# jaronlong52/neuron_poker

Hardware: NVIDIA B200
Metric: showdown_evals_per_s (higher is better)
Workload: dtype u32

## Files before the change

neuron_poker_b200/csrc/npk_device.cuh:

```cuda
#pragma once
#include <cuda_runtime.h>
#include <stdint.h>

namespace npk {

constexpr int kDevDescShift = 9;
constexpr int kRowBits = 10;
constexpr uint32_t kColMask = (1u << kRowBits) - 1u;

struct DeviceTables {
    const uint16_t* value;
    const uint16_t* rowoff;
    const uint16_t* flush;
    const uint32_t* desc;
    uint32_t value_bytes;
    uint32_t rowoff_bytes;
    uint32_t flush_bytes;
    uint16_t type_start[10];
    uint32_t* check;
};

struct SmemTables {
    const uint16_t* value;
    const uint16_t* rowoff;
    const uint16_t* flush;
    const uint32_t* desc;
    uint32_t value_bytes, rowoff_bytes, flush_bytes;
    uint32_t* check;
};

#ifdef NPK_CHECKED
#define NPK_CHECK(ptr, cond, code) do { if (!(cond)) atomicMax((ptr), (unsigned)(code)); } while (0)
#else
#define NPK_CHECK(ptr, cond, code) do { } while (0)
#endif

constexpr uint32_t kDescBytes = 256;

__device__ __forceinline__ uint32_t smem_u32(const void* p) { return (uint32_t)__cvta_generic_to_shared(p); }

__device__ __forceinline__ void mbar_init(uint64_t* bar, uint32_t count)
{
    asm volatile("mbarrier.init.shared::cta.b64 [%0], %1;" ::"r"(smem_u32(bar)), "r"(count));
    asm volatile("fence.mbarrier_init.release.cluster;" ::: "memory");
}
__device__ __forceinline__ void mbar_expect_tx(uint64_t* bar, uint32_t bytes)
{
    asm volatile("mbarrier.arrive.expect_tx.shared::cta.b64 _, [%0], %1;" ::"r"(smem_u32(bar)), "r"(bytes) : "memory");
}
__device__ __forceinline__ void bulk_g2s(void* dst, const void* src, uint32_t bytes, uint64_t* bar)
{
    asm volatile("cp.async.bulk.shared::cluster.global.mbarrier::complete_tx::bytes [%0], [%1], %2, [%3];" ::"r"(
                     smem_u32(dst)),
                 "l"(src), "r"(bytes), "r"(smem_u32(bar))
                 : "memory");
}
__device__ __forceinline__ void mbar_wait(uint64_t* bar, uint32_t parity)
{
    uint32_t done = 0;
    while (!done) {
        asm volatile(
            "{\n .reg .pred p;\n mbarrier.try_wait.parity.shared::cta.b64 p, [%1], %2;\n selp.u32 %0, 1, 0, p;\n}\n"
            : "=r"(done)
            : "r"(smem_u32(bar)), "r"(parity)
            : "memory");
    }
}

__device__ __forceinline__ SmemTables stage_tables(const DeviceTables& t, uint8_t* base, uint64_t* bar)
{
    uint8_t* s_value = base;
    uint8_t* s_rowoff = s_value + t.value_bytes;
    uint8_t* s_flush = s_rowoff + t.rowoff_bytes;
    if (threadIdx.x == 0) mbar_init(bar, 1);
    __syncthreads();
    if (threadIdx.x == 0) {
        mbar_expect_tx(bar, t.value_bytes + t.rowoff_bytes + t.flush_bytes + kDescBytes);
        const uint32_t kChunk = 32768;
        for (uint32_t o = 0; o < t.value_bytes; o += kChunk)
            bulk_g2s(s_value + o, (const uint8_t*)t.value + o, min(kChunk, t.value_bytes - o), bar);
        bulk_g2s(s_rowoff, t.rowoff, t.rowoff_bytes, bar);
        bulk_g2s(s_flush, t.flush, t.flush_bytes, bar);
        bulk_g2s(s_flush + t.flush_bytes, t.desc, kDescBytes, bar);
    }
    mbar_wait(bar, 0);
    SmemTables s;
    s.value = (const uint16_t*)s_value;
    s.rowoff = (const uint16_t*)s_rowoff;
    s.flush = (const uint16_t*)s_flush;
    s.desc = (const uint32_t*)(s_flush + t.flush_bytes);
    s.value_bytes = t.value_bytes; s.rowoff_bytes = t.rowoff_bytes; s.flush_bytes = t.flush_bytes; s.check = t.check;
    return s;
}

__device__ __forceinline__ void philox4x32_10(uint32_t c0, uint32_t c1, uint32_t c2, uint32_t c3, uint32_t k0,
                                              uint32_t k1, uint32_t out[4])
{
    const uint32_t M0 = 0xD2511F53u, M1 = 0xCD9E8D57u, W0 = 0x9E3779B9u, W1 = 0xBB67AE85u;
#pragma unroll
    for (int r = 0; r < 10; r++) {
        uint64_t p0 = (uint64_t)M0 * c0, p1 = (uint64_t)M1 * c2;
        uint32_t n0 = (uint32_t)(p1 >> 32) ^ c1 ^ k0;
        uint32_t n2 = (uint32_t)(p0 >> 32) ^ c3 ^ k1;
        c1 = (uint32_t)p1;
        c3 = (uint32_t)p0;
        c0 = n0;
        c2 = n2;
        k0 += W0;
        k1 += W1;
    }
    out[0] = c0; out[1] = c1; out[2] = c2; out[3] = c3;
}

__device__ __forceinline__ uint32_t prmt(uint32_t a, uint32_t b, uint32_t sel)
{
    uint32_t r;
    asm("prmt.b32 %0, %1, %2, %3;" : "=r"(r) : "r"(a), "r"(b), "r"(sel));
    return r;
}

__device__ __forceinline__ uint32_t shr_clamp(uint32_t v, uint32_t n)
{
    uint32_t r;
    asm("shr.u32 %0, %1, %2;" : "=r"(r) : "r"(v), "r"(n));
    return r;
}

__device__ __forceinline__ uint32_t lds_u16(uint32_t saddr)
{
    uint32_t v;
    asm("ld.shared.u16 %0, [%1];" : "=r"(v) : "r"(saddr));
    return v;
}

struct SmemAddr {
    uint32_t value, rowoff, flush;
#ifdef NPK_CHECKED
    uint32_t value_bytes, rowoff_bytes, flush_bytes;
    uint32_t* check;
#endif
};

__device__ __forceinline__ SmemAddr smem_addr(const SmemTables& s)
{
    SmemAddr a;
    a.value = smem_u32(s.value); a.rowoff = smem_u32(s.rowoff); a.flush = smem_u32(s.flush);
#ifdef NPK_CHECKED
    a.value_bytes = s.value_bytes; a.rowoff_bytes = s.rowoff_bytes; a.flush_bytes = s.flush_bytes; a.check = s.check;
#endif
    return a;
}

__device__ __forceinline__ uint32_t lookup_nonflush(const SmemAddr& a, uint32_t total)
{
    const uint32_t row2 = __umulhi(total, 1u << (32 - (kDevDescShift + kRowBits - 1))) & (0xFFFFu << 1);
    NPK_CHECK(a.check, row2 + 2u <= a.rowoff_bytes, 1);
    const uint32_t off = lds_u16(a.rowoff + row2);
    const uint32_t col2 = __umulhi(total, 1u << (32 - (kDevDescShift - 1))) & (kColMask << 1);
    NPK_CHECK(a.check, col2 + (off << 1) + 2u <= a.value_bytes, 2);
    return lds_u16(a.value + col2 + (off << 1));
}

__device__ __forceinline__ uint32_t flush_bit(uint32_t d, uint32_t fsx) { return shr_clamp(0x1000u, (d ^ fsx) & 63u); }

__device__ __forceinline__ void card_bits(uint32_t d, uint32_t& lo, uint32_t& hi)
{
    const uint64_t b = 1ull << ((d & 0x30u) + 12u - (d & 15u));
    lo = (uint32_t)b;
    hi = (uint32_t)(b >> 32);
}

__device__ __forceinline__ uint32_t suit_inc(uint32_t d) { return 1u << ((d >> 2) & 12u); }

__device__ __forceinline__ uint32_t field_selector(uint32_t fs) { return 0x9910u + fs * 0x2222u; }

__device__ __forceinline__ uint32_t eval7_desc(const SmemAddr& a, const uint32_t d[7])
{
    uint32_t total = 0, cnt = 0x3333u;
#pragma unroll
    for (int i = 0; i < 7; i++) {
        total += d[i];
        cnt += suit_inc(d[i]);
    }
    uint32_t v = lookup_nonflush(a, total);
    const uint32_t f = cnt & 0x8888u;
    if (f) {
        const uint32_t fsx = (((31u - __clz(f)) >> 2) & 3u) << 4;
        uint32_t field = 0;
#pragma unroll
        for (int i = 0; i < 7; i++) field |= shr_clamp(0x1000u, (d[i] ^ fsx) & 63u);
        NPK_CHECK(a.check, 2u * field + 2u <= a.flush_bytes, 3);
        v = lds_u16(a.flush + 2u * field);
    }
    return v;
}

}
```

neuron_poker_b200/csrc/npk_mc.cuh:

```cuda
#pragma once
#include "npk_device.cuh"
#include "npk_kernels.h"

namespace npk {

__device__ __forceinline__ long long next_item(unsigned long long* counter, int lane)
{
    unsigned long long it = 0;
    if (lane == 0) it = atomicAdd(counter, 1ull);
    return (long long)__shfl_sync(0xffffffffu, it, 0);
}

__device__ __forceinline__ void item_range(const EquityParams& p, long long item, long long& qslot, long long& begin, long long& end)
{
    qslot = item / p.chunks;
    begin = (item - qslot * p.chunks) * p.chunk;
    end = min(p.trials, begin + (long long)p.chunk);
}

struct QueryStatic {
    uint32_t hero_sum;
    uint32_t hero_lo, hero_hi;
    uint32_t board_sum;
    uint32_t board_lo, board_hi;
    uint32_t board_cnt;
    uint64_t known;
};

__device__ __forceinline__ QueryStatic load_query(const EquityParams& p, const uint32_t* sdesc, long long q, int nb_known)
{
    QueryStatic s;
    const uint8_t h0 = p.hole ? p.hole[2 * q] : (uint8_t)p.inline_query;
    const uint8_t h1 = p.hole ? p.hole[2 * q + 1] : (uint8_t)(p.inline_query >> 8);
    uint32_t d0 = sdesc[h0], d1 = sdesc[h1], l, h;
    s.hero_sum = d0 + d1;
    card_bits(d0, s.hero_lo, s.hero_hi);
    card_bits(d1, l, h);
    s.hero_lo |= l; s.hero_hi |= h;
    s.known = (1ull << h0) | (1ull << h1);
    s.board_sum = 0; s.board_lo = 0; s.board_hi = 0; s.board_cnt = 0x5555u;
    for (int i = 0; i < nb_known; i++) {
        const uint8_t c = p.hole ? p.board[5 * q + i] : (uint8_t)(p.inline_query >> (16 + 8 * i));
        uint32_t d = sdesc[c];
        card_bits(d, l, h);
        s.board_sum += d; s.board_lo |= l; s.board_hi |= h; s.board_cnt += suit_inc(d);
        s.known |= 1ull << c;
    }
    return s;
}

__device__ __forceinline__ void finish_single_call(const EquityParams& p, int lane)
{
    SingleCall* sc = p.single;
    if (!sc) return;
    __syncwarp();
    unsigned int last = 0;
    if (lane == 0) {
        __threadfence();
        const unsigned int total = gridDim.x * (blockDim.x >> 5);
        last = atomicAdd(&sc->ticket, 1u) == total - 1u;
    }
    last = __shfl_sync(0xffffffffu, last, 0);
    if (!last) return;
    __threadfence();
    unsigned long long v = 0;
    if (lane < 12) {
        unsigned long long* src = &sc->wins;
        v = atomicExch(src + lane, 0ull);
    }
    if (lane == 0) { sc->work_counter = 0; sc->ticket = 0; }
    if (p.single_quick) {
        const unsigned long long t = __shfl_sync(0xffffffffu, v, 1);
        if (lane == 0) {
            const uint4 q = make_uint4((unsigned int)v, (unsigned int)t, (unsigned int)p.single_seq, (unsigned int)(p.single_seq >> 32));
            asm volatile("st.global.v4.u32 [%0], {%1, %2, %3, %4};" ::"l"(&sc->host->quick), "r"(q.x), "r"(q.y), "r"(q.z), "r"(q.w)
                         : "memory");
        }
        return;
    }
    if (lane < 12) (&sc->host->wins)[lane] = v;
    __threadfence_system();
    __syncwarp();
    if (lane == 0) *reinterpret_cast<volatile unsigned long long*>(&sc->host->seq) = p.single_seq;
}

static __device__ __noinline__ void finish_peer(PeerCall* pc, unsigned long long epoch, unsigned long long* totals, uint32_t words,
                                         int lane)
{
    __syncwarp();
    unsigned int last = 0;
    if (lane == 0) {
        __threadfence();
        const unsigned int total = gridDim.x * (blockDim.x >> 5);
        last = atomicAdd(&pc->ticket, 1u) == total - 1u;
    }
    last = __shfl_sync(0xffffffffu, last, 0);
    if (!last) return;
    __threadfence();
    const uint32_t world = pc->world, me = pc->rank;
    const uint32_t parity = (uint32_t)(epoch & 1ull);
    const size_t my_slot = ((size_t)parity * world + me) * pc->stride;
    for (uint32_t base = 0; base < words; base += 128) {
        unsigned long long v[4];
#pragma unroll
        for (int k = 0; k < 4; k++) {
            const uint32_t i = base + 32u * k + lane;
            v[k] = i < words ? atomicExch(&pc->acc[i], 0ull) : 0ull;
        }
        for (uint32_t r = 0; r < world; r++) {
            unsigned long long* dst = pc->slots[r] + my_slot;
#pragma unroll
            for (int k = 0; k < 4; k++) {
                const uint32_t i = base + 32u * k + lane;
                if (i < words) dst[i] = v[k];
            }
        }
    }
    __threadfence_system();
    __syncwarp();
    if (lane < world)
        asm volatile("st.release.sys.global.u64 [%0], %1;" ::"l"(pc->flags[lane] + parity * kMaxPeers + me), "l"(epoch) : "memory");
    if (lane < world) {
        const unsigned long long* f = pc->flags[me] + parity * kMaxPeers + lane;
        const long long t0 = clock64();
        unsigned long long seen;
        for (;;) {
            asm volatile("ld.acquire.sys.global.u64 %0, [%1];" : "=l"(seen) : "l"(f) : "memory");
            if (seen >= epoch) break;
            if (clock64() - t0 > (4ll << 30)) { pc->error = 1u; break; }
        }
    }
    __syncwarp();
    const unsigned long long* mine = pc->slots[me] + (size_t)parity * world * pc->stride;
    for (uint32_t base = 0; base < words; base += 128) {
        unsigned long long sum[4] = {0, 0, 0, 0};
#pragma unroll 4
        for (uint32_t r = 0; r < world; r++) {
#pragma unroll
            for (int k = 0; k < 4; k++) {
                const uint32_t i = base + 32u * k + lane;
                if (i < words) sum[k] += __ldcg(mine + (size_t)r * pc->stride + i);
            }
        }
#pragma unroll
        for (int k = 0; k < 4; k++) {
            const uint32_t i = base + 32u * k + lane;
            if (i < words) totals[i] = sum[k];
        }
    }
    if (lane == 0) { pc->work_counter = 0; pc->ticket = 0; }
}

struct BoardFlush {
    uint32_t fsx;
    uint32_t sel;
    uint32_t thr;
};

__device__ __forceinline__ BoardFlush board_flush(uint32_t board_cnt)
{
    BoardFlush b;
    const uint32_t f = board_cnt & 0x8888u;
    const uint32_t fs = ((31u - __clz(f)) >> 2) & 3u;
    b.fsx = fs << 4;
    b.sel = field_selector(fs);
    b.thr = f ? 5u : 64u;
    return b;
}

__device__ __forceinline__ uint32_t eval_player(const SmemAddr& a, uint32_t total, uint32_t field, uint32_t thr)
{
    uint32_t v = lookup_nonflush(a, total);
    NPK_CHECK(a.check, 2u * field + 2u <= a.flush_bytes, 3);
    if ((uint32_t)__popc(field) >= thr) v = max(v, lds_u16(a.flush + 2u * field));
    return v;
}

__device__ __forceinline__ uint32_t lds_u32(uint32_t saddr)
{
    uint32_t v;
    asm volatile("ld.shared.u32 %0, [%1];" : "=r"(v) : "r"(saddr) : "memory");
    return v;
}
__device__ __forceinline__ void sts_u32(uint32_t saddr, uint32_t v)
{
    asm volatile("st.shared.u32 [%0], %1;" ::"r"(saddr), "r"(v) : "memory");
}

struct WarpCtx {
    SmemAddr st;
    const uint32_t* sdesc;
    uint32_t* scratch;
    uint32_t fy_addr;
    int lane;
};

__device__ __forceinline__ WarpCtx warp_context(const EquityParams& p, uint8_t* smem, int words_per_warp)
{
    uint64_t* bar = reinterpret_cast<uint64_t*>(smem);
    const SmemTables stab = stage_tables(p.tables, smem + 128, bar);
    const uint32_t table_bytes = 128 + p.tables.value_bytes + p.tables.rowoff_bytes + p.tables.flush_bytes + kDescBytes;
    const int warp = threadIdx.x >> 5, lane = threadIdx.x & 31;
    WarpCtx cx;
    cx.st = smem_addr(stab);
    cx.sdesc = stab.desc;
    cx.scratch = reinterpret_cast<uint32_t*>(smem + table_bytes) + warp * words_per_warp;
    cx.fy_addr = smem_u32(cx.scratch + 64 + lane);
    cx.lane = lane;
    return cx;
}

template <int NOPP, int NB>
__device__ __forceinline__ void uniform_item(const EquityParams& p, const WarpCtx& cx, long long q, long long t_begin,
            long long t_end)
{
    constexpr int KNOWN = 5 - NB;
    constexpr int N = 50 - KNOWN;
    constexpr int D = 2 * NOPP + NB;
    constexpr int NW = (D + 1) / 2;
    constexpr int NBLK2 = (2 * NW + 3) / 4;
    static_assert(D <= N, "not enough cards");

    const SmemAddr& st = cx.st;
    const int lane = cx.lane;
    uint32_t* scratch = cx.scratch;
    uint32_t* fy = scratch + 64 + lane;
    const uint32_t fy_addr = cx.fy_addr;
    const QueryStatic qs = load_query(p, cx.sdesc, q, KNOWN);

    __syncwarp();
    {
        const uint64_t avail = ~qs.known & ((1ull << 52) - 1ull);
        for (int c = lane; c < 52; c += 32)
            if (avail >> c & 1ull) scratch[__popcll(avail & ((1ull << c) - 1ull))] = cx.sdesc[c];
    }
    __syncwarp();
#pragma unroll 4
    for (int j = 0; j < N; j++) fy[j * 32] = scratch[j];
    __syncwarp();

    const unsigned long long a_begin = (unsigned long long)(p.trial_offset + t_begin);
    const unsigned long long a_end = (unsigned long long)(p.trial_offset + t_end);
    uint32_t wins = 0, ties = 0;
    unsigned long long wt_pack = 0;

    const uint32_t span = (uint32_t)(a_end - a_begin);
    uint32_t rel = (uint32_t)(2ull * (a_begin >> 1) - a_begin) + 2u * (uint32_t)lane;
    for (unsigned long long pb = a_begin >> 1; pb <= (a_end - 1) >> 1; pb += 32, rel += 64u) {
        const unsigned long long pair = pb + lane;
        uint32_t w[NBLK2 > 0 ? NBLK2 * 4 : 1];
#pragma unroll
        for (int b = 0; b < NBLK2; b++)
            philox4x32_10((uint32_t)pair, (uint32_t)(pair >> 32), (uint32_t)q + p.query_offset, (uint32_t)b,
                          p.seed_lo, p.seed_hi, &w[4 * b]);
        uint32_t dv[2][D > 0 ? D : 1];
#pragma unroll
        for (int u = 0; u < 2; u++) {
            uint32_t slot[D > 0 ? D : 1];
            uint32_t rem = 0;
#pragma unroll
            for (int k = 0; k < D; k++) {
                const uint32_t x = (k & 1) ? rem : w[u * NW + (k >> 1)];
                const uint32_t idx = __umulhi(x, (uint32_t)(N - k));
                rem = x * (uint32_t)(N - k);
                slot[k] = fy_addr + idx * 128u;
                dv[u][k] = lds_u32(slot[k]);
                sts_u32(slot[k], lds_u32(fy_addr + (uint32_t)(N - 1 - k) * 128u));
            }
#pragma unroll
            for (int k = D - 1; k >= 0; k--) sts_u32(slot[k], dv[u][k]);
        }
#pragma unroll
        for (int u = 0; u < 2; u++) {
            const bool active = rel + (uint32_t)u < span;
            uint32_t bsum = qs.board_sum, bcnt = qs.board_cnt;
#pragma unroll
            for (int k = 2 * NOPP; k < D; k++) { bsum += dv[u][k]; bcnt += suit_inc(dv[u][k]); }
            const BoardFlush bf = board_flush(bcnt);
            uint32_t bfield = prmt(qs.board_lo, qs.board_hi, bf.sel);
#pragma unroll
            for (int k = 2 * NOPP; k < D; k++) bfield |= flush_bit(dv[u][k], bf.fsx);
            const uint32_t hv = eval_player(st, bsum + qs.hero_sum, bfield | prmt(qs.hero_lo, qs.hero_hi, bf.sel), bf.thr);
            uint32_t best = 0;
#pragma unroll
            for (int o = 0; o < NOPP; o++) {
                const uint32_t d0 = dv[u][2 * o], d1 = dv[u][2 * o + 1];
                best = max(best, eval_player(st, bsum + d0 + d1, bfield | flush_bit(d0, bf.fsx) | flush_bit(d1, bf.fsx), bf.thr));
            }
            const bool win = active && (NOPP == 0 || hv > best), tie = active && NOPP > 0 && hv == best;
            wins += win; ties += tie;
            if (p.win_types && (win || tie)) {
                uint32_t ty = 0;
#pragma unroll
                for (int i = 1; i < 9; i++) ty += hv >= p.tables.type_start[i];
                wt_pack += 1ull << (7 * ty);
            }
        }
    }
#ifdef NPK_CHECKED
    __syncwarp();
    for (int j = 0; j < N; j++) NPK_CHECK(st.check, fy[j * 32] == scratch[j], 7);
#endif
    wins = __reduce_add_sync(0xffffffffu, wins);
    ties = __reduce_add_sync(0xffffffffu, ties);
    if (lane == 0) {
        atomicAdd(&p.wins[q], (unsigned long long)wins);
        atomicAdd(&p.ties[q], (unsigned long long)ties);
    }
    if (p.win_types) {
#pragma unroll
        for (int i = 0; i < 9; i++) {
            uint32_t c = __reduce_add_sync(0xffffffffu, (uint32_t)(wt_pack >> (7 * i)) & 127u);
            if (lane == 0 && c) atomicAdd(&p.win_types[9 * q + i], (unsigned long long)c);
        }
    }
}


struct WordStream {
    uint32_t c0, c1, c2, k0, k1, blk, have;
    uint32_t w[4];
    __device__ __forceinline__ uint32_t next()
    {
        if (have == 0) { philox4x32_10(c0, c1, c2, blk++, k0, k1, w); have = 4; }
        const uint32_t r = w[0];
        w[0] = w[1]; w[1] = w[2]; w[2] = w[3];
        have--;
        return r;
    }
};

__device__ __forceinline__ int select_bit(uint64_t m, int k)
{
    uint32_t lo = (uint32_t)m, hi = (uint32_t)(m >> 32);
    int c = __popc(lo), base = 0;
    uint32_t w = lo;
    if (k >= c) { k -= c; w = hi; base = 32; }
#pragma unroll
    for (int s = 16; s >= 1; s >>= 1) {
        const uint32_t lowmask = (1u << s) - 1u;
        const int cl = __popc(w & lowmask);
        if (k >= cl) { k -= cl; w >>= s; base += s; } else { w &= lowmask; }
    }
    return base;
}

#ifndef NPK_IMAD_LEVEL
#define NPK_IMAD_LEVEL 0
#endif
static __constant__ uint32_t c_mul[12] = {1u, 256u, 65536u, 1u << 24, 1u << 25, 128u, 1u << 31, 1u << 23, 1u << 15, 0u, 0u, 0u};

__device__ __forceinline__ uint32_t imad_lo(uint32_t a, uint32_t b, uint32_t c)
{
    uint32_t r;
    asm("mad.lo.u32 %0, %1, %2, %3;" : "=r"(r) : "r"(a), "r"(b), "r"(c));
    return r;
}
__device__ __forceinline__ uint32_t imad_hi(uint32_t a, uint32_t b, uint32_t c)
{
    uint32_t r;
    asm("mad.hi.u32 %0, %1, %2, %3;" : "=r"(r) : "r"(a), "r"(b), "r"(c));
    return r;
}

__device__ __forceinline__ uint32_t bump4(uint32_t x4, uint32_t c, uint32_t h)
{
#if NPK_IMAD_LEVEL >= 2
    const uint32_t t = imad_lo(x4, c_mul[0], c) & h;
#else
    const uint32_t t = (x4 + c) & h;
#endif
#if NPK_IMAD_LEVEL >= 1
    return imad_hi(t, c_mul[4], x4);
#else
    return x4 + (t >> 7);
#endif
}

template <int D>
__device__ __forceinline__ void lehmer_decode(const uint32_t (&raw)[D > 0 ? D : 1], uint32_t (&x4)[(D + 3) / 4 > 0 ? (D + 3) / 4 : 1])
{
    constexpr int G = (D + 3) / 4;
#pragma unroll
    for (int g = 0; g < G; g++) {
        uint32_t v = raw[4 * g];
#pragma unroll
        for (int b = 1; b < 4; b++)
            if (4 * g + b < D) {
#if NPK_IMAD_LEVEL >= 1
                v = imad_lo(raw[4 * g + b], c_mul[b], v);
#else
                v += raw[4 * g + b] << (8 * b);
#endif
            }
        x4[g] = v;
    }
#pragma unroll
    for (int k = D - 2; k >= 0; k--) {
        const uint32_t c = 0x80808080u - raw[k] * 0x01010101u;
#pragma unroll
        for (int g = (k + 1) / 4; g < G; g++) {
            uint32_t h = 0;
#pragma unroll
            for (int b = 0; b < 4; b++)
                if (4 * g + b > k && 4 * g + b < D) h |= 0x80u << (8 * b);
            x4[g] = bump4(x4[g], c, h);
        }
    }
}

__device__ __forceinline__ uint32_t slot_addr(uint32_t x4, int b, uint32_t base)
{
    const uint32_t f = x4 & (0xFFu << (8 * b));
#if NPK_IMAD_LEVEL >= 1
    return b == 0 ? imad_lo(f, c_mul[5], base) : imad_hi(f, c_mul[5 + b], base);
#else
    return b == 0 ? base + f * 128u : base + (f >> (8 * b - 7));
#endif
}

template <int NOPP, int NB>
__device__ __forceinline__ void refdeal_item(const EquityParams& p, const WarpCtx& cx, long long q, long long t_begin,
            long long t_end)
{
    constexpr int KNOWN = 5 - NB;
    constexpr int N = 50 - KNOWN;
    constexpr int D = 2 * NOPP + NB;
#ifdef NPK_UNIFORM_LEHMER
    constexpr int NWR = (D + 1) / 2;
#else
    constexpr int NWR = NOPP + (NB + 1) / 2;
#endif
    constexpr int NBLK2 = (2 * NWR + 3) / 4;
    constexpr int G = (D + 3) / 4;
    static_assert(D <= N, "not enough cards");

    const SmemAddr& st = cx.st;
    const int lane = cx.lane;
    uint32_t* scratch = cx.scratch;
    uint32_t* fy = scratch + 64 + lane;
    const uint32_t fy_addr = cx.fy_addr;
    const QueryStatic qs = load_query(p, cx.sdesc, q, KNOWN);

    __syncwarp();
    {
        const uint64_t avail = ~qs.known & ((1ull << 52) - 1ull);
        for (int c = lane; c < 52; c += 32)
            if (avail >> c & 1ull) scratch[__popcll(avail & ((1ull << c) - 1ull))] = cx.sdesc[c];
    }
    __syncwarp();
#pragma unroll 4
    for (int j = 0; j < N; j++) fy[j * 32] = scratch[j];
    __syncwarp();

    const unsigned long long a_begin = (unsigned long long)(p.trial_offset + t_begin);
    const unsigned long long a_end = (unsigned long long)(p.trial_offset + t_end);
    uint32_t wins = 0, ties = 0, passes = 0;
    unsigned long long wt_pack = 0;

    const uint32_t span = (uint32_t)(a_end - a_begin);
    uint32_t rel = (uint32_t)(2ull * (a_begin >> 1) - a_begin) + 2u * (uint32_t)lane;
    for (unsigned long long pb = a_begin >> 1; pb <= (a_end - 1) >> 1; pb += 32, rel += 64u) {
        const unsigned long long pair = pb + lane;
        uint32_t w[NBLK2 > 0 ? NBLK2 * 4 : 1];
#pragma unroll
        for (int b = 0; b < NBLK2; b++)
            philox4x32_10((uint32_t)pair, (uint32_t)(pair >> 32), (uint32_t)q + p.query_offset, 0x80000000u + (uint32_t)b,
                          p.seed_lo, p.seed_hi, &w[4 * b]);
        uint32_t dv[2][D > 0 ? D : 1];
#pragma unroll
        for (int u = 0; u < 2; u++) {
            uint32_t raw[D > 0 ? D : 1];
#ifdef NPK_UNIFORM_LEHMER
            {
                uint32_t remw = 0;
#pragma unroll
                for (int k = 0; k < D; k++) {
                    const uint32_t x = (k & 1) ? remw : w[u * NWR + (k >> 1)];
                    raw[k] = __umulhi(x, (uint32_t)(N - k));
                    remw = x * (uint32_t)(N - k);
                }
            }
#else
#pragma unroll
            for (int o = 0; o < NOPP; o++) {
                const uint32_t m = (uint32_t)(N - 2 * o - 1);
                const uint32_t x = w[u * NWR + o];
                const uint32_t a = __umulhi(x, m), b = __umulhi(x * m, m);
                raw[2 * o] = a + (a >= b ? 1u : 0u);
                raw[2 * o + 1] = b;
            }
            uint32_t rem = 0;
#pragma unroll
            for (int c = 0; c < NB; c++) {
                const uint32_t m = (uint32_t)(N - 2 * NOPP - c - 1);
                const uint32_t x = (c & 1) ? rem : w[u * NWR + NOPP + (c >> 1)];
                raw[2 * NOPP + c] = __umulhi(x, m);
                rem = x * m;
            }
#endif
            uint32_t x4[G > 0 ? G : 1];
            lehmer_decode<D>(raw, x4);
#pragma unroll
            for (int k = 0; k < D; k++) dv[u][k] = lds_u32(slot_addr(x4[k >> 2], k & 3, fy_addr));
        }
        if (p.passes) {
            constexpr int NPB = (2 * NOPP + 3) / 4;
#pragma unroll
            for (int b = 0; b < NPB; b++) {
                uint32_t pw[4];
                philox4x32_10((uint32_t)pair, (uint32_t)(pair >> 32), (uint32_t)q + p.query_offset, 0x40000000u + (uint32_t)b,
                              p.seed_lo, p.seed_hi, pw);
#pragma unroll
                for (int i = 0; i < 4; i++) {
                    const int s = 4 * b + i;
                    if (s < 2 * NOPP) {
                        const uint32_t n = (uint32_t)(N - 2 * (s % (NOPP > 0 ? NOPP : 1)));
                        uint32_t x = pw[i], tries = 1;
                        while (x < 0xFFFFFFFFu / n && tries < kMaxRangeAttempts) { tries++; x *= n; }
                        if (rel + (uint32_t)(s / (NOPP > 0 ? NOPP : 1)) < span) passes += tries;
                    }
                }
            }
        }
#pragma unroll
        for (int u = 0; u < 2; u++) {
            const bool active = rel + (uint32_t)u < span;
            uint32_t bsum = qs.board_sum, bcnt = qs.board_cnt;
#pragma unroll
            for (int k = 2 * NOPP; k < D; k++) { bsum += dv[u][k]; bcnt += suit_inc(dv[u][k]); }
            const BoardFlush bf = board_flush(bcnt);
            uint32_t bfield = prmt(qs.board_lo, qs.board_hi, bf.sel);
#pragma unroll
            for (int k = 2 * NOPP; k < D; k++) bfield |= flush_bit(dv[u][k], bf.fsx);
            const uint32_t hv = eval_player(st, bsum + qs.hero_sum, bfield | prmt(qs.hero_lo, qs.hero_hi, bf.sel), bf.thr);
            uint32_t best = 0;
#pragma unroll
            for (int o = 0; o < NOPP; o++) {
                const uint32_t d0 = dv[u][2 * o], d1 = dv[u][2 * o + 1];
                best = max(best, eval_player(st, bsum + d0 + d1, bfield | flush_bit(d0, bf.fsx) | flush_bit(d1, bf.fsx), bf.thr));
            }
            const bool win = active && (NOPP == 0 || hv > best), tie = active && NOPP > 0 && hv == best;
            wins += win; ties += tie;
            if (p.win_types && (win || tie)) {
                uint32_t ty = 0;
#pragma unroll
                for (int i = 1; i < 9; i++) ty += hv >= p.tables.type_start[i];
                wt_pack += 1ull << (7 * ty);
            }
        }
    }

    wins = __reduce_add_sync(0xffffffffu, wins);
    ties = __reduce_add_sync(0xffffffffu, ties);
    if (lane == 0) {
        atomicAdd(&p.wins[q], (unsigned long long)wins);
        atomicAdd(&p.ties[q], (unsigned long long)ties);
    }
    if (p.passes) {
        const uint32_t plo = __reduce_add_sync(0xffffffffu, passes & 0xffffu);
        const uint32_t phi = __reduce_add_sync(0xffffffffu, passes >> 16);
        if (lane == 0) atomicAdd(&p.passes[q], (unsigned long long)plo + ((unsigned long long)phi << 16));
    }
    if (p.win_types) {
#pragma unroll
        for (int i = 0; i < 9; i++) {
            uint32_t c = __reduce_add_sync(0xffffffffu, (uint32_t)(wt_pack >> (7 * i)) & 127u);
            if (lane == 0 && c) atomicAdd(&p.win_types[9 * q + i], (unsigned long long)c);
        }
    }
}


}
```

Before: 452.1 billion.

## Skip opponent evaluations once hero is beaten and trim Fisher-Yates restore stores

Moves the showdown logic into a templated helper. In the main Monte Carlo path, opponents from the third onward are evaluated with predicated shared-memory loads that are suppressed once an earlier opponent already beats the hero, since the result can no longer change. The liveness check is refreshed only every two opponents to keep the loads batched. The Fisher-Yates swap/restore also drops the redundant last-slot store and reuses a cached tail value instead of reloading it, at the cost of extra predicate logic per evaluation.

Result: faster. 461.3 billion (median of 6 runs) (+2.0%).

```diff
diff --git a/neuron_poker_b200/csrc/npk_device.cuh b/neuron_poker_b200/csrc/npk_device.cuh
--- a/neuron_poker_b200/csrc/npk_device.cuh
+++ b/neuron_poker_b200/csrc/npk_device.cuh
@@ -133,6 +133,13 @@
     return v;
 }
 
+__device__ __forceinline__ uint32_t lds_u16_if(uint32_t saddr, bool live, uint32_t other)
+{
+    uint32_t v = other;
+    asm("{\n .reg .pred p;\n setp.ne.u32 p, %2, 0;\n @p ld.shared.u16 %0, [%1];\n}" : "+r"(v) : "r"(saddr), "r"((uint32_t)live));
+    return v;
+}
+
 struct SmemAddr {
     uint32_t value, rowoff, flush;
 #ifdef NPK_CHECKED
diff --git a/neuron_poker_b200/csrc/npk_mc.cuh b/neuron_poker_b200/csrc/npk_mc.cuh
--- a/neuron_poker_b200/csrc/npk_mc.cuh
+++ b/neuron_poker_b200/csrc/npk_mc.cuh
@@ -176,6 +176,54 @@
     return v;
 }
 
+__device__ __forceinline__ uint32_t eval_player_if(const SmemAddr& a, uint32_t total, uint32_t field, uint32_t thr, bool live)
+{
+    const uint32_t row2 = __umulhi(total, 1u << (32 - (kDevDescShift + kRowBits - 1))) & (0xFFFFu << 1);
+    NPK_CHECK(a.check, row2 + 2u <= a.rowoff_bytes, 1);
+    const uint32_t off = lds_u16_if(a.rowoff + row2, live, row2);
+    const uint32_t col2 = __umulhi(total, 1u << (32 - (kDevDescShift - 1))) & (kColMask << 1);
+    NPK_CHECK(a.check, !live || col2 + (off << 1) + 2u <= a.value_bytes, 2);
+    const uint32_t voff = col2 + (off << 1);
+    uint32_t v = lds_u16_if(a.value + voff, live, voff);
+    NPK_CHECK(a.check, 2u * field + 2u <= a.flush_bytes, 3);
+    if (live && (uint32_t)__popc(field) >= thr) v = max(v, lds_u16(a.flush + 2u * field));
+    return v;
+}
+
+template <int NOPP, int NB, bool EARLY_OUT>
+__device__ __forceinline__ void showdown(const EquityParams& p, const SmemAddr& st, const QueryStatic& qs,
+                                         const uint32_t (&dv)[2 * NOPP + NB > 0 ? 2 * NOPP + NB : 1], bool active,
+                                         uint32_t& wins, uint32_t& ties, unsigned long long& wt_pack)
+{
+    constexpr int D = 2 * NOPP + NB;
+    uint32_t bsum = qs.board_sum, bcnt = qs.board_cnt;
+#pragma unroll
+    for (int k = 2 * NOPP; k < D; k++) { bsum += dv[k]; bcnt += suit_inc(dv[k]); }
+    const BoardFlush bf = board_flush(bcnt);
+    uint32_t bfield = prmt(qs.board_lo, qs.board_hi, bf.sel);
+#pragma unroll
+    for (int k = 2 * NOPP; k < D; k++) bfield |= flush_bit(dv[k], bf.fsx);
+    const uint32_t hv = eval_player(st, bsum + qs.hero_sum, bfield | prmt(qs.hero_lo, qs.hero_hi, bf.sel), bf.thr);
+    uint32_t best = 0;
+    bool live = true;
+#pragma unroll
+    for (int o = 0; o < NOPP; o++) {
+        const uint32_t d0 = dv[2 * o], d1 = dv[2 * o + 1];
+        const uint32_t total = bsum + d0 + d1, field = bfield | flush_bit(d0, bf.fsx) | flush_bit(d1, bf.fsx);
+        const bool staged = EARLY_OUT && o >= 2;
+        if (staged && o % 2 == 0) live = best <= hv;
+        best = max(best, staged ? eval_player_if(st, total, field, bf.thr, live) : eval_player(st, total, field, bf.thr));
+    }
+    const bool win = active && (NOPP == 0 || hv > best), tie = active && NOPP > 0 && hv == best;
+    wins += win; ties += tie;
+    if (p.win_types && (win || tie)) {
+        uint32_t ty = 0;
+#pragma unroll
+        for (int i = 1; i < 9; i++) ty += hv >= p.tables.type_start[i];
+        wt_pack += 1ull << (7 * ty);
+    }
+}
+
 __device__ __forceinline__ uint32_t lds_u32(uint32_t saddr)
 {
     uint32_t v;
@@ -238,6 +286,7 @@
 #pragma unroll 4
     for (int j = 0; j < N; j++) fy[j * 32] = scratch[j];
     __syncwarp();
+    const uint32_t tail0 = scratch[N - 1];
 
     const unsigned long long a_begin = (unsigned long long)(p.trial_offset + t_begin);
     const unsigned long long a_end = (unsigned long long)(p.trial_offset + t_end);
@@ -265,37 +314,13 @@
                 rem = x * (uint32_t)(N - k);
                 slot[k] = fy_addr + idx * 128u;
                 dv[u][k] = lds_u32(slot[k]);
-                sts_u32(slot[k], lds_u32(fy_addr + (uint32_t)(N - 1 - k) * 128u));
-            }
-#pragma unroll
-            for (int k = D - 1; k >= 0; k--) sts_u32(slot[k], dv[u][k]);
-        }
-#pragma unroll
-        for (int u = 0; u < 2; u++) {
-            const bool active = rel + (uint32_t)u < span;
-            uint32_t bsum = qs.board_sum, bcnt = qs.board_cnt;
-#pragma unroll
-            for (int k = 2 * NOPP; k < D; k++) { bsum += dv[u][k]; bcnt += suit_inc(dv[u][k]); }
-            const BoardFlush bf = board_flush(bcnt);
-            uint32_t bfield = prmt(qs.board_lo, qs.board_hi, bf.sel);
-#pragma unroll
-            for (int k = 2 * NOPP; k < D; k++) bfield |= flush_bit(dv[u][k], bf.fsx);
-            const uint32_t hv = eval_player(st, bsum + qs.hero_sum, bfield | prmt(qs.hero_lo, qs.hero_hi, bf.sel), bf.thr);
-            uint32_t best = 0;
-#pragma unroll
-            for (int o = 0; o < NOPP; o++) {
-                const uint32_t d0 = dv[u][2 * o], d1 = dv[u][2 * o + 1];
-                best = max(best, eval_player(st, bsum + d0 + d1, bfield | flush_bit(d0, bf.fsx) | flush_bit(d1, bf.fsx), bf.thr));
-            }
-            const bool win = active && (NOPP == 0 || hv > best), tie = active && NOPP > 0 && hv == best;
-            wins += win; ties += tie;
-            if (p.win_types && (win || tie)) {
-                uint32_t ty = 0;
-#pragma unroll
-                for (int i = 1; i < 9; i++) ty += hv >= p.tables.type_start[i];
-                wt_pack += 1ull << (7 * ty);
-            }
-        }
+                if (k < D - 1) sts_u32(slot[k], k == 0 ? tail0 : lds_u32(fy_addr + (uint32_t)(N - 1 - k) * 128u));
+            }
+#pragma unroll
+            for (int k = D - 2; k >= 0; k--) sts_u32(slot[k], dv[u][k]);
+        }
+#pragma unroll
+        for (int u = 0; u < 2; u++) showdown<NOPP, NB, true>(p, st, qs, dv[u], rel + (uint32_t)u < span, wins, ties, wt_pack);
     }
 #ifdef NPK_CHECKED
     __syncwarp();
@@ -524,31 +549,7 @@
             }
         }
 #pragma unroll
-        for (int u = 0; u < 2; u++) {
-            const bool active = rel + (uint32_t)u < span;
-            uint32_t bsum = qs.board_sum, bcnt = qs.board_cnt;
-#pragma unroll
-            for (int k = 2 * NOPP; k < D; k++) { bsum += dv[u][k]; bcnt += suit_inc(dv[u][k]); }
-            const BoardFlush bf = board_flush(bcnt);
-            uint32_t bfield = prmt(qs.board_lo, qs.board_hi, bf.sel);
-#pragma unroll
-            for (int k = 2 * NOPP; k < D; k++) bfield |= flush_bit(dv[u][k], bf.fsx);
-            const uint32_t hv = eval_player(st, bsum + qs.hero_sum, bfield | prmt(qs.hero_lo, qs.hero_hi, bf.sel), bf.thr);
-            uint32_t best = 0;
-#pragma unroll
-            for (int o = 0; o < NOPP; o++) {
-                const uint32_t d0 = dv[u][2 * o], d1 = dv[u][2 * o + 1];
-                best = max(best, eval_player(st, bsum + d0 + d1, bfield | flush_bit(d0, bf.fsx) | flush_bit(d1, bf.fsx), bf.thr));
-            }
-            const bool win = active && (NOPP == 0 || hv > best), tie = active && NOPP > 0 && hv == best;
-            wins += win; ties += tie;
-            if (p.win_types && (win || tie)) {
-                uint32_t ty = 0;
-#pragma unroll
-                for (int i = 1; i < 9; i++) ty += hv >= p.tables.type_start[i];
-                wt_pack += 1ull << (7 * ty);
-            }
-        }
+        for (int u = 0; u < 2; u++) showdown<NOPP, NB, false>(p, st, qs, dv[u], rel + (uint32_t)u < span, wins, ties, wt_pack);
     }
 
     wins = __reduce_add_sync(0xffffffffu, wins);
```
